# mpeg5/xevd

Hardware: AMD Instinct MI355X
Metric: frames/sec (bit-exact YUV) + achieved HBM GB/s (higher is better)
Workload: dtype s16; 1 GPU; cfg4_main_8k_10b_ra; width=7680, height=4320, bit_depth=10, batches_resident=4, residual_pass_ahead=True, parallelism=1 stream on 1 GPU

## Files before the change

xevd_amd/csrc/k_inter.hip:

```cpp
#include "xgpu_internal.h"

#include <hip/hip_ext.h>
#include <type_traits>
#include "mc_filters.h"

#define LDS_AS __attribute__((address_space(3)))

#define UW_STRIDE 48
#define UI_STRIDE 40
#define UC_STRIDE 24
#define UCW_STRIDE 32
static_assert(UI_STRIDE <= UW_STRIDE && UC_STRIDE <= UCW_STRIDE, "an intermediate row is not longer than the window row it replaces");
#define UT_L_SAMPLES (40 * UW_STRIDE)
#define UT_C_SAMPLES (3 * 64 * 8)
#define UNI_SAMPLES   (UT_L_SAMPLES + UT_C_SAMPLES)
static_assert(2 * 19 * UCW_STRIDE <= UT_C_SAMPLES, "both chroma windows fit");

__device__ __forceinline__ void wave_lds_sync()
{
    __builtin_amdgcn_fence(__ATOMIC_RELEASE, "wavefront");
    __builtin_amdgcn_wave_barrier();
    __builtin_amdgcn_fence(__ATOMIC_ACQUIRE, "wavefront");
}

// ... 93 lines not shown
                const uint2 a = w[0], b = w[1];
                E[0] = a.x; E[1] = a.y; E[2] = b.x; E[3] = b.y;
            }
            uint2 r;
            if (H) {
                const uint32_t O[3] = { hi_lo(E[1], E[0]), hi_lo(E[2], E[1]), hi_lo(E[3], E[2]) };
                int t[4];
                if (SH && odd) {
                    t[0] = dot2(ch[1], O[1], dot2z(ch[0], O[0]));
                    t[1] = dot2(ch[1], E[2], dot2z(ch[0], E[1]));
                    t[2] = dot2(ch[1], O[2], dot2z(ch[0], O[1]));
                    t[3] = dot2(ch[1], E[3], dot2z(ch[0], E[2]));
                } else {
                    t[0] = dot2(ch[1], E[1], dot2z(ch[0], E[0]));
                    t[1] = dot2(ch[1], O[1], dot2z(ch[0], O[0]));
                    t[2] = dot2(ch[1], E[2], dot2z(ch[0], E[1]));
                    t[3] = dot2(ch[1], O[2], dot2z(ch[0], O[1]));
                }
#pragma unroll
                for (int q = 0; q < 4; q++) { t[q] >>= rg.sh1; if (!V) t[q] = clip3(0, maxv, t[q]); }
                r = make_uint2(pack2(t[0], t[1]), pack2(t[2], t[3]));
            } else {
                if (SH && odd) r = make_uint2(E[1], E[2]);
                else r = make_uint2(hi_lo(E[1], E[0]), hi_lo(E[2], E[1]));
            }
            *(uint2 *)(I + prow * UC_STRIDE + 4 * g) = r;
        }
    }
    wave_lds_sync();
#pragma unroll
    for (int pl = 0; pl < 2; pl++) {
        const int16_t *base = I + (pl * 19 + ((lane >> 3) << 1)) * UC_STRIDE + ((lane & 7) << 1);
        uint32_t *o = pl ? ov : ou;
        if (!V) {
            o[0] = *(const uint32_t *)(base + UC_STRIDE); o[1] = *(const uint32_t *)(base + 2 * UC_STRIDE);
        } else {
            uint32_t q[5];
#pragma unroll
            for (int j = 0; j < 5; j++) q[j] = *(const uint32_t *)(base + j * UC_STRIDE);
            int acc[2][2];
#pragma unroll
            for (int j = 1; j < 5; j++) {
                const uint32_t pr[2] = { __builtin_amdgcn_perm(q[j], q[j - 1], 0x05040100u), __builtin_amdgcn_perm(q[j], q[j - 1], 0x07060302u) };
#pragma unroll
                for (int c = 0; c < 2; c++)
#pragma unroll
                    for (int r = 0; r < 2; r++) {
                        const int d = j - 1 - r;
                        if (d == 0) acc[r][c] = dot2a(cv[0], pr[c], rg.off2);
                        else if (d == 2) acc[r][c] = dot2(cv[1], pr[c], acc[r][c]);
                    }
            }
#pragma unroll
            for (int r = 0; r < 2; r++)
                o[r] = pack2(clip3(0, maxv, acc[r][0] >> rg.sh2), clip3(0, maxv, acc[r][1] >> rg.sh2));
        }
    }
    wave_lds_sync();
}
#define REG_W_STRIDE 80
#define REG_C_STRIDE 48
#define REG_W_SAMPLES (71 * REG_W_STRIDE)
#define REG_C_SAMPLES (35 * REG_C_STRIDE)
#define REG_I_SAMPLES (39 * UI_STRIDE)
#define REG_SAMPLES   (REG_W_SAMPLES + 2 * REG_C_SAMPLES + 4 * REG_I_SAMPLES)
struct RegionMap { int y[3], c[2]; };
__device__ __forceinline__ RegionMap region_map(int t)
{
    RegionMap m;
#pragma unroll
    for (int it = 0; it < 3; it++) {
        const int idx = t + 256 * it, row = idx / 10, k = idx - row * 10;
        m.y[it] = idx < 71 * 10 ? (row << 8) | k : -1;
    }
#pragma unroll
    for (int it = 0; it < 2; it++) {
        const int idx = t + 256 * it, pl = idx >= 210, j = idx - 210 * pl, row = j / 6, k = j - row * 6;
        m.c[it] = idx < 420 ? (row << 8) | (pl << 7) | k : -1;
    }
    return m;
}

template <bool H, bool V>
__device__ __forceinline__ void mc_scu_list(gs16 pl_, int s_l, gs16 pu_, gs16 pv_, int s_c, const uint32_t ch[4], const uint32_t cv[4], Regime rgl, int maxl,
                                            const uint32_t c2h[2], const uint32_t c2v[2], Regime rgc, int maxc, bool cwh, bool cwv, uint32_t o[8], uint32_t ou[2], uint32_t ov[2],
                                            bool fx, bool fy, bool cfx, bool cfy)
{
    constexpr int J0 = V ? 0 : 3, J1 = V ? 11 : 7;
#ifdef XGPU_NO_LANE_PRED
    fx = fy = cfx = cfy = true;
#endif
    v4u32 A[11]; v2u32 B[11];
    auto request = [&](int ja, int jb) {
#pragma unroll
        for (int j = ja; j < jb; j++) {
            const bool row_on = !V || fy || (j >= 3 && j < 7);
            if (H) {
                A[j] = any_value<v4u32>(); B[j] = any_value<v2u32>();
                gload16_if(A[j], pl_ + j * s_l, row_on);
                gload8_if(B[j], pl_ + j * s_l + 8, row_on && fx);
            } else {
                B[j] = any_value<v2u32>();
                gload8_if(B[j], pl_ + j * s_l + 3, row_on);
            }
        }
    };
    auto fence = [&](int ja, int jb) {
#pragma unroll
        for (int j = ja; j < jb; j++) {
            if (H) asm volatile("" : "+v"(A[j]), "+v"(B[j]));
            else   asm volatile("" : "+v"(B[j]));
        }
    };
    int acc[4][4];
    int tp[4] = {0, 0, 0, 0};
    auto row = [&](int j) {
        int t[4];
        if (H) {
            const uint32_t D0 = A[j].x, D1 = A[j].y, D2 = A[j].z, D3 = A[j].w, D4 = B[j].x, D5 = B[j].y;
            const uint32_t Q0 = hi_lo(D1, D0), Q1 = hi_lo(D2, D1), Q2 = hi_lo(D3, D2), Q3 = hi_lo(D4, D3), Q4 = hi_lo(D5, D4);
            t[0] = dot2(ch[3], D3, dot2(ch[2], D2, dot2(ch[1], D1, dot2z(ch[0], D0))));
            t[2] = dot2(ch[3], D4, dot2(ch[2], D3, dot2(ch[1], D2, dot2z(ch[0], D1))));
            t[1] = dot2(ch[3], Q3, dot2(ch[2], Q2, dot2(ch[1], Q1, dot2z(ch[0], Q0))));
            t[3] = dot2(ch[3], Q4, dot2(ch[2], Q3, dot2(ch[1], Q2, dot2z(ch[0], Q1))));
#pragma unroll
            for (int c = 0; c < 4; c++) t[c] = clip3(rgl.lo1, rgl.hi1, t[c] >> rgl.sh1);
        } else {
            t[0] = (int)(int16_t)(B[j].x & 0xFFFF); t[1] = (int)(int16_t)(B[j].x >> 16);
            t[2] = (int)(int16_t)(B[j].y & 0xFFFF); t[3] = (int)(int16_t)(B[j].y >> 16);
        }
        if (!V) {
#pragma unroll
            for (int c = 0; c < 4; c++) acc[j - 3][c] = t[c];
            return;
        }
        if (j > 0) {
#pragma unroll
            for (int c = 0; c < 4; c++) {
                const uint32_t pr = pack2(tp[c], t[c]);
#pragma unroll
                for (int r = 0; r < 4; r++) {
                    const int d = j - 1 - r;
                    if (d == 0) acc[r][c] = dot2a(cv[0], pr, rgl.off2);
                    else if (d > 0 && d <= 6 && (d & 1) == 0) acc[r][c] = dot2(cv[d >> 1], pr, acc[r][c]);
                }
            }
        }
#pragma unroll
        for (int c = 0; c < 4; c++) tp[c] = t[c];
    };
    auto rows = [&](int ja, int jb) {
#pragma unroll
        for (int j = ja; j < jb; j++) row(j);
    };
    auto luma_out = [&]() {
#pragma unroll
        for (int r = 0; r < 4; r++) {
            int v[4];
#pragma unroll
            for (int c = 0; c < 4; c++) v[c] = clip3(0, maxl, V ? acc[r][c] >> rgl.sh2 : acc[r][c]);
            o[r * 2 + 0] = pack2(v[0], v[1]);
            o[r * 2 + 1] = pack2(v[2], v[3]);
        }
    };
    v3u32 CW[2][5];
    auto request_c = [&](int pl) {
#pragma unroll
        for (int j = 0; j < 5; j++) {
            const bool row_on = cfy || j == 1 || j == 2;
            CW[pl][j] = any_value<v3u32>();
            gload12_if(CW[pl][j], (pl ? pv_ : pu_) + j * s_c, row_on);
        }
    };
    auto fence_c = [&](int pl) {
#pragma unroll
        for (int j = 0; j < 5; j++) asm volatile("" : "+v"(CW[pl][j]));
    };
    auto chroma = [&](auto hc, auto vc, int pl, uint32_t oo[2]) {
        constexpr bool CH = decltype(hc)::value, CV = decltype(vc)::value;
        int a2[2][2];
        int tq[2] = {0, 0};
#pragma unroll
        for (int j = CV ? 0 : 1; j < (CV ? 5 : 3); j++) {
            int t[2];
            const uint32_t D0 = CW[pl][j].x, D1 = CW[pl][j].y, D2 = CW[pl][j].z;
            if (CH) {
                const uint32_t Q0 = hi_lo(D1, D0), Q1 = hi_lo(D2, D1);
                t[0] = dot2(c2h[1], D1, dot2z(c2h[0], D0));
                t[1] = dot2(c2h[1], Q1, dot2z(c2h[0], Q0));
#pragma unroll
                for (int c = 0; c < 2; c++) t[c] = clip3(rgc.lo1, rgc.hi1, t[c] >> rgc.sh1);
            } else {
                const uint32_t q = hi_lo(D1, D0);
                t[0] = (int)(int16_t)(q & 0xFFFF); t[1] = (int)(int16_t)(q >> 16);
            }
            if (!CV) { a2[j - 1][0] = t[0]; a2[j - 1][1] = t[1]; continue; }
            if (j > 0) {
#pragma unroll
                for (int c = 0; c < 2; c++) {
                    const uint32_t pr = pack2(tq[c], t[c]);
#pragma unroll
                    for (int r = 0; r < 2; r++) {
                        const int d = j - 1 - r;
                        if (d == 0) a2[r][c] = dot2a(c2v[0], pr, rgc.off2);
                        else if (d == 2) a2[r][c] = dot2(c2v[1], pr, a2[r][c]);
                    }
                }
            }
            tq[0] = t[0]; tq[1] = t[1];
        }
#pragma unroll
        for (int r = 0; r < 2; r++)
            oo[r] = pack2(clip3(0, maxc, CV ? a2[r][0] >> rgc.sh2 : a2[r][0]), clip3(0, maxc, CV ? a2[r][1] >> rgc.sh2 : a2[r][1]));
    };
    using T = std::true_type; using F = std::false_type;
    auto chroma_pl = [&](int pl, uint32_t oo[2]) {
        fence_c(pl);
        if (cwh) { if (cwv) chroma(T{}, T{}, pl, oo); else chroma(T{}, F{}, pl, oo); }
        else     { if (cwv) chroma(F{}, T{}, pl, oo); else chroma(F{}, F{}, pl, oo); }
    };
    request(J0, J1); fence(J0, J1);
    rows(J0, J1);
    luma_out();
    __builtin_amdgcn_sched_barrier(0);
    request_c(0); request_c(1);
    chroma_pl(0, ou); chroma_pl(1, ov);
}

#define OWNER_NONE 0xFFFFFFFFu

#ifdef XGPU_INTER_TRACE
__device__ unsigned long long g_inter_trace[3][16];
struct InterTrace { unsigned long long prev; int role; bool on; };
#define TRACE_MARK(tr, p) do { if ((tr).on) { const unsigned long long now_ = __builtin_amdgcn_s_memtime(); atomicAdd(&g_inter_trace[(tr).role][p], now_ - (tr).prev); (tr).prev = __builtin_amdgcn_s_memtime(); } } while (0)
#define TRACE_ARG , InterTrace &tr
#define TRACE_PASS , tr
#define TRACE_OFF InterTrace tr = { 0, 0, false };
extern "C" int xgpu_test_inter_trace(unsigned long long out[48], int reset)
{
    if (hipMemcpyFromSymbol(out, HIP_SYMBOL(g_inter_trace), sizeof(g_inter_trace)) != hipSuccess) return -1;
    if (reset) { static unsigned long long z[48]; if (hipMemcpyToSymbol(HIP_SYMBOL(g_inter_trace), z, sizeof(z)) != hipSuccess) return -1; }
    return 0;
}
#else
#define TRACE_MARK(tr, p) do { } while (0)
#define TRACE_ARG
#define TRACE_PASS
#define TRACE_OFF
#endif
template <int MODE>
__device__ __forceinline__ bool inter_tile(const InterArgs &a, uint4 r0, uint4 r1, bool lane_ok, int sx, int sy, int lane, int16_t *W, const LaneMap fm,
                                           const uint4 (*s_ref)[2], const uint4 *s_ltap, const uint2 *s_ctap, uint32_t pl[8], uint32_t pu[2], uint32_t pv[2],
                                           const RegionMap *rm, int wave, uint32_t own TRACE_ARG)
{
    constexpr bool UNI = MODE != 0;
    if (UNI) {
        own = (uint32_t)__builtin_amdgcn_readfirstlane((int)own);
        r0.x = __builtin_amdgcn_readfirstlane(r0.x); r0.y = __builtin_amdgcn_readfirstlane(r0.y); r0.z = __builtin_amdgcn_readfirstlane(r0.z); r0.w = __builtin_amdgcn_readfirstlane(r0.w);
        r1.x = __builtin_amdgcn_readfirstlane(r1.x); r1.y = __builtin_amdgcn_readfirstlane(r1.y); r1.z = __builtin_amdgcn_readfirstlane(r1.z); r1.w = __builtin_amdgcn_readfirstlane(r1.w);
    } else if (!lane_ok) return false;
    const int cu_x = r0.x & 0xFFFF, cu_y = r0.x >> 16;
    const int lw = r0.y & 0xFF, lh = (r0.y >> 8) & 0xFF, pred_mode = (r0.y >> 16) & 0xF, cbf = r0.y >> 24;
    const int refi0 = (int)(int8_t)(r0.z & 0xFF), refi1 = (int)(int8_t)((r0.z >> 8) & 0xFF), qp_map = (r0.z >> 16) & 0xFF;
    const uint32_t coef_off = r0.w;
    const int cw = 1 << lw, chh = 1 << lh;
    const int x = sx << 2, y = sy << 2;
    const bool intra = pred_mode == XGPU_MODE_INTRA;
    const int ai = (intra || pred_mode == XGPU_MODE_IBC) ? 0 : (int)((r1.w >> 8) & 0xFF);
    int tu_x = 0, tu_y = 0, tu_w = cw, tu_h = chh;
    if (ai) {
        const int idx = ai & 15, pos = ai >> 4;
        if (idx == 2 || idx == 4) { tu_h = chh >> (idx == 4 ? 2 : 1); tu_y = pos ? chh - tu_h : 0; }
        else                      { tu_w = cw >> (idx == 3 ? 2 : 1);  tu_x = pos ? cw - tu_w : 0; }
    }
    const int lx = x - cu_x - tu_x, ly = y - cu_y - tu_y;
    const bool in_tu = (uint32_t)lx < (uint32_t)tu_w && (uint32_t)ly < (uint32_t)tu_h;

    {
        uint32_t m = ((uint32_t)qp_map << 16) | ((uint32_t)intra << 15) | (1u << 31);
        m |= SCU_RANK(own);
        if (pred_mode == XGPU_MODE_SKIP) m |= 1u << 23;
        const bool ibc = pred_mode == XGPU_MODE_IBC;
        if (ibc) m |= 1u << 26;
        if (((r0.z >> 24) & 1) && in_tu) m |= 1u << 24;
        if (((x - cu_x) & 63) == 0) m |= SCU_EDGE_L;
        if (((y - cu_y) & 63) == 0) m |= SCU_EDGE_T;
        if (x == cu_x && ((r0.y >> 16) & CU_NOCH_L)) m |= SCU_NOCH_L;
        if (y == cu_y && ((r0.y >> 16) & CU_NOCH_T)) m |= SCU_NOCH_T;
        uint4 rec;
        rec.x = m;
        rec.y = (intra || ibc) ? 0x0000FFFFu : ((r0.z & 0xFFFFu) | ((uint32_t)ai << 16));
        rec.z = intra ? 0u : r1.x;
        rec.w = (intra || ibc) ? 0u : r1.y;
        bool other0 = false, other1 = false;
        if (!intra && !ibc) {
            if ((r1.w >> 16) & 0xFF) { other0 = refi0 >= 0; other1 = refi1 >= 0; }
            else if (a.dmvr_to_map && (r1.w >> 24)) {
                const int q0 = refi0 >= 0 ? (int)s_ref[refi0 * 2][1].z : 0, q1 = refi1 >= 0 ? (int)s_ref[refi1 * 2 + 1][1].z : 0;
                other0 = other1 = dmvr_applies(a.cur_poc, q0, q1);
            }
        }
        ScuRec *const mp = &a.maps[sy * a.w_scu + sx];
        if (!other0 && !other1) *(uint4 *)mp = rec;
        else {
            *(uint2 *)mp = make_uint2(rec.x, rec.y);
            if (!other0) ((uint32_t *)mp)[2] = rec.z;
// ... 109 lines not shown
                    const int idx = lane + 64 * it, plane = idx >= 76, j = idx - 76 * plane;
                    if (idx < 152 && wanted(j >> 2, j & 3)) __builtin_amdgcn_global_load_lds((const GAS void *)((plane ? rv_ : ru_) + off + (j >> 2) * a.s_c + 8 * (j & 3)), (LDS_AS void *)(d + it * 1024), 16, 0, 0);
                }
            }
        };
        constexpr int N_LUMA_REQ = REGION ? 3 : 4, N_CHROMA_REQ = REGION ? 2 : 3;
        const int l_first = use[0] ? 0 : 1, n_lists = (int)use[0] + (int)use[1];
        TRACE_MARK(tr, 2);
        load_resid();
        if (n_lists) { request_luma(l_first); __builtin_amdgcn_sched_barrier(0); request_chroma(l_first); }
        TRACE_MARK(tr, 3);
#pragma unroll 1
        for (int i = 0; i < n_lists; i++) {
            const int l = i ? 1 : l_first;
            const bool more = i + 1 < n_lists;
            int px, py;
            list_pos(l, px, py);
            const int mvx = l ? mvs[1][0] : mvs[0][0], mvy = l ? mvs[1][1] : mvs[0][1];
            const int ldx = (mvx & 3) != 0, ldy = (mvy & 3) != 0, cdx = (mvx & 7) != 0, cdy = (mvy & 7) != 0;
            uint32_t o[8], ou[2], ov[2];
            if (REGION) { asm volatile("s_waitcnt vmcnt(0)" ::: "memory"); __syncthreads(); }
            else { asm volatile("s_waitcnt vmcnt(%0)" :: "n"(N_CHROMA_REQ) : "memory"); wave_lds_sync(); }
            TRACE_MARK(tr, i ? 8 : 4);
            {
                const uint4 th = s_ltap[ldx ? ((px & 3) << 2) : 16], tv = s_ltap[ldy ? ((py & 3) << 2) : 16];
                const uint32_t ch[4] = { th.x, th.y, th.z, th.w }, cv[4] = { tv.x, tv.y, tv.z, tv.w };
                const Regime rg = regime(ldx, ldy, a.bd_l);
                const int mis = ((px >> 2) - 3) & 7, odd = mis & 1;
                const int16_t *const Wy = Wy0 + (mis & ~1);
                if (ldx) { if (ldy) luma_tile_filter<true, true, WS_L, true>(Wy, ch, cv, rg, maxl, I, lane, o, odd); else luma_tile_filter<true, false, WS_L, true>(Wy, ch, cv, rg, maxl, I, lane, o, odd); }
                else     { if (ldy) luma_tile_filter<false, true, WS_L, true>(Wy, ch, cv, rg, maxl, I, lane, o, odd); else luma_tile_filter<false, false, WS_L, true>(Wy, ch, cv, rg, maxl, I, lane, o, odd); }
            }
            TRACE_MARK(tr, 5);
            if (more) {
                if (REGION) __syncthreads(); else wave_lds_sync();
                request_luma(1);
            }
            if (!REGION) {
                if (more) asm volatile("s_waitcnt vmcnt(%0)" :: "n"(N_LUMA_REQ) : "memory"); else asm volatile("s_waitcnt vmcnt(0)" ::: "memory");
                wave_lds_sync();
            }
            TRACE_MARK(tr, 6);
            {
                const uint2 th = s_ctap[cdx ? ((px & 7) << 2) : 32], tv = s_ctap[cdy ? ((py & 7) << 2) : 32];
                const uint32_t c2h[2] = { th.x, th.y }, c2v[2] = { tv.x, tv.y };
                const Regime rg = regime(cdx, cdy, a.bd_c);
                const int mis = ((px >> 3) - 1) & 7, odd = mis & 1;
                const int16_t *const Wu = Wu0 + (mis & ~1), *const Wv = Wu + C_SAMPLES;
                if (cdx) { if (cdy) chroma_tile_filter<true, true, WS_C, true>(Wu, Wv, c2h, c2v, rg, maxc, IC, lane, ou, ov, odd); else chroma_tile_filter<true, false, WS_C, true>(Wu, Wv, c2h, c2v, rg, maxc, IC, lane, ou, ov, odd); }
                else     { if (cdy) chroma_tile_filter<false, true, WS_C, true>(Wu, Wv, c2h, c2v, rg, maxc, IC, lane, ou, ov, odd); else chroma_tile_filter<false, false, WS_C, true>(Wu, Wv, c2h, c2v, rg, maxc, IC, lane, ou, ov, odd); }
            }
            TRACE_MARK(tr, 7);
            if (more) {
                if (REGION) __syncthreads(); else wave_lds_sync();
                request_chroma(1);
            }
            if (nl == 0) {
#pragma unroll
                for (int k = 0; k < 8; k++) pl[k] = o[k];
                pu[0] = ou[0]; pu[1] = ou[1]; pv[0] = ov[0]; pv[1] = ov[1];
            } else {
#pragma unroll
                for (int k = 0; k < 8; k++) pl[k] = avg2(pl[k], o[k]);
                pu[0] = avg2(pu[0], ou[0]); pu[1] = avg2(pu[1], ou[1]);
                pv[0] = avg2(pv[0], ov[0]); pv[1] = avg2(pv[1], ov[1]);
            }
            nl++;
        }
        (void)tid;
    } else {
        TRACE_MARK(tr, 2);
#pragma unroll
        for (int l = 0; l < 2; l++) {
            if (!use[l]) continue;
            const uint4 e0 = s_ref[refis[l] * 2 + l][0], e1 = s_ref[refis[l] * 2 + l][1];
            const gs16 ry_ = (gs16)(((uint64_t)e0.y << 32) | e0.x), ru_ = (gs16)(((uint64_t)e0.w << 32) | e0.z), rv_ = (gs16)(((uint64_t)e1.y << 32) | e1.x);
            const int mvx = mvs[l][0], mvy = mvs[l][1];
            const int px = (x << 2) + mvt[l][0], py = (y << 2) + mvt[l][1];
            const int ldx = (mvx & 3) != 0, ldy = (mvy & 3) != 0;
            const int cdx = (mvx & 7) != 0, cdy = (mvy & 7) != 0;
            uint32_t ch[4], cv[4], o[8], ou[2], ov[2];
            {
                const uint4 th = s_ltap[ldx ? ((px & 3) << 2) : 16], tv = s_ltap[ldy ? ((py & 3) << 2) : 16];
                ch[0] = th.x; ch[1] = th.y; ch[2] = th.z; ch[3] = th.w; cv[0] = tv.x; cv[1] = tv.y; cv[2] = tv.z; cv[3] = tv.w;
                const uint2 cth = s_ctap[cdx ? ((px & 7) << 2) : 32], ctv = s_ctap[cdy ? ((py & 7) << 2) : 32];
                const uint32_t c2h[2] = { cth.x, cth.y }, c2v[2] = { ctv.x, ctv.y };
                const gs16 p = ry_ + ((py >> 2) - 3) * a.s_l + (px >> 2) - 3;
                const int off = ((py >> 3) - 1) * a.s_c + (px >> 3) - 1;
                const Regime rgl = regime(ldx, ldy, a.bd_l), rgc = regime(cdx, cdy, a.bd_c);
                const bool wh = __ballot(ldx) != 0, wvv = __ballot(ldy) != 0;
                const bool cwh = __ballot(cdx) != 0, cwv = __ballot(cdy) != 0;
#define MC_S(H, V) mc_scu_list<H, V>(p, a.s_l, ru_ + off, rv_ + off, a.s_c, ch, cv, rgl, maxl, c2h, c2v, rgc, maxc, cwh, cwv, o, ou, ov, ldx != 0, ldy != 0, cdx != 0, cdy != 0)
                if (wh) { if (wvv) MC_S(true, true); else MC_S(true, false); }
                else    { if (wvv) MC_S(false, true); else MC_S(false, false); }
#undef MC_S
            }
            if (nl == 0) {
#pragma unroll
                for (int k = 0; k < 8; k++) pl[k] = o[k];
                pu[0] = ou[0]; pu[1] = ou[1]; pv[0] = ov[0]; pv[1] = ov[1];
            } else {
#pragma unroll
                for (int k = 0; k < 8; k++) pl[k] = avg2(pl[k], o[k]);
                pu[0] = avg2(pu[0], ou[0]); pu[1] = avg2(pu[1], ou[1]);
                pv[0] = avg2(pv[0], ov[0]); pv[1] = avg2(pv[1], ov[1]);
            }
            nl++;
        }
    }
    TRACE_MARK(tr, 9);
    if (MODE == 0) load_resid();
    if (nl == 0) return false;

    if (cbf & 1) {
#pragma unroll
        for (int k = 0; k < 8; k++) pl[k] = recon2(pl[k], rl[k], maxl);
    }
    if (cbf & 2) { pu[0] = recon2(pu[0], ru[0], maxl); pu[1] = recon2(pu[1], ru[1], maxl); }
    if (cbf & 4) { pv[0] = recon2(pv[0], rv[0], maxl); pv[1] = recon2(pv[1], rv[1], maxl); }

    return true;
}

__device__ __forceinline__ int xcd_slice(int block, int grid) { return (block & 7) * (grid >> 3) + (block >> 3); }

__device__ __forceinline__ void store_scu(const InterArgs &a, int sx, int sy, const uint32_t pl[8], const uint32_t pu[2], const uint32_t pv[2])
{
    const int x = sx << 2, y = sy << 2;
    int16_t *dy = a.cur_y + y * a.s_l + x;
#pragma unroll
    for (int k = 0; k < 4; k++) *(uint2 *)(dy + k * a.s_l) = make_uint2(pl[k * 2], pl[k * 2 + 1]);
    const int coff = (y >> 1) * a.s_c + (x >> 1);
    *(uint32_t *)(a.cur_u + coff) = pu[0];
    *(uint32_t *)(a.cur_u + coff + a.s_c) = pu[1];
    *(uint32_t *)(a.cur_v + coff) = pv[0];
    *(uint32_t *)(a.cur_v + coff + a.s_c) = pv[1];
}
#define ARG_REFS(a)  ((const uint4 (*)[2])&(a).refp[0][0])
#define ARG_LTAPS(a) ((const uint4 *)&k_luma_taps[(a).admvp][0][0])
#define ARG_CTAPS(a) ((const uint2 *)&k_chroma_taps[(a).admvp][0][0])
static_assert(sizeof(RefEntry) == 32, "a reference entry is two 16-byte halves");
static_assert(XGPU_INTER_STRIP == 16, "the strip arithmetic below shifts by four");

struct SplitTables { uint4 ref[XGPU_MAX_REFS * 2][2]; uint4 ltap[17]; uint2 ctap[33]; uint2 pad; };

__device__ __forceinline__ void inter_fused_body(const InterArgs &a)
{
    __shared__ __attribute__((aligned(16))) int16_t s_win[REG_SAMPLES];
    static_assert(4 * UNI_SAMPLES <= REG_SAMPLES, "the four waves' tile blocks fit into the region block");
    __shared__ SplitTables s_tab[4];
    const int idx = xcd_slice(blockIdx.x, gridDim.x);
    if (idx >= a.n_work) return;
    const int t = threadIdx.x, lane = t & 63, wave = __builtin_amdgcn_readfirstlane(t >> 6);
#ifdef XGPU_INTER_TRACE
    InterTrace tr = { __builtin_amdgcn_s_memtime(), 0, lane == 0 && (idx % 61) == 7 };
#endif
    int rx, ry;
    if (idx < a.full_entries) {
        const int s = (int)__umulhi((uint32_t)idx, a.magic_strip), r = idx - s * a.strip_entries;
        ry = r >> 4; rx = (s << 4) + (r & 15);
    } else {
        const int r = idx - a.full_entries;
        ry = a.magic_last ? (int)__umulhi((uint32_t)r, a.magic_last) : r; rx = (a.regions_x & ~15) + r - ry * (a.regions_x & 15);
    }
    const int sx = (rx << 4) + ((wave & 1) << 3) + (lane & 7), sy = (ry << 4) + ((wave >> 1) << 3) + (lane >> 3);
    const uint32_t kinds = a.work[idx];
    const uint4 *const item = (const uint4 *)&a.items[idx * 4 + wave];
    const uint4 e = item[0], i0 = item[1], i1 = item[2];
    const uint32_t own = (sx < (a.pic_w >> 2) && sy < (a.pic_h >> 2)) ? a.owner[sy * a.w_scu + sx] : OWNER_NONE;
    const LaneMap fm0 = { 0, 0 };
    uint32_t pl[8], pu[2], pv[2];
    if (kinds == XGPU_WORK_REGION) {
// ... 117 lines not shown
```

xevd_amd/csrc/mc_filters.h:

```cpp
#pragma once
#include "xgpu_internal.h"

typedef short v2s __attribute__((ext_vector_type(2)));
struct __attribute__((packed, aligned(2))) U32x4u { uint32_t a, b, c, d; };
struct __attribute__((packed, aligned(2))) U32x2u { uint32_t a, b; };
struct __attribute__((packed, aligned(2))) U32x1u { uint32_t a; };
#define GAS __attribute__((address_space(1)))
typedef const GAS int16_t *gs16;
typedef uint32_t v4u32 __attribute__((ext_vector_type(4)));
typedef uint32_t v2u32 __attribute__((ext_vector_type(2)));
typedef uint32_t v3u32 __attribute__((ext_vector_type(3)));
typedef v4u32 __attribute__((aligned(2))) v4u32_u;
typedef v2u32 __attribute__((aligned(2))) v2u32_u;
typedef v3u32 __attribute__((aligned(2))) v3u32_u;
typedef uint32_t __attribute__((aligned(2))) u32_u;
__device__ __forceinline__ uint4 gload16(gs16 p) { const v4u32 v = *(const GAS v4u32_u *)p; return make_uint4(v.x, v.y, v.z, v.w); }
__device__ __forceinline__ uint2 gload8(gs16 p) { const v2u32 v = *(const GAS v2u32_u *)p; return make_uint2(v.x, v.y); }
__device__ __forceinline__ uint32_t gload4(gs16 p) { return *(const GAS u32_u *)p; }
template <typename T> __device__ __forceinline__ T any_value() { T v; asm volatile("" : "=v"(v)); return v; }
__device__ __forceinline__ void gload16_if(v4u32 &v, gs16 p, bool on) { if (on) v = *(const GAS v4u32_u *)p; }
__device__ __forceinline__ void gload8_if(v2u32 &v, gs16 p, bool on) { if (on) v = *(const GAS v2u32_u *)p; }
__device__ __forceinline__ void gload12_if(v3u32 &v, gs16 p, bool on) { if (on) v = *(const GAS v3u32_u *)p; }
__device__ __forceinline__ void gload4_if(uint32_t &v, gs16 p, bool on) { if (on) v = *(const GAS u32_u *)p; }

__device__ __forceinline__ int dot2(uint32_t a, uint32_t b, int c)
{
    return __builtin_amdgcn_sdot2(__builtin_bit_cast(v2s, a), __builtin_bit_cast(v2s, b), c, false);
}
__device__ __forceinline__ int dot2z(uint32_t a, uint32_t b)
{
    int r;
    asm("v_dot2_i32_i16 %0, %1, %2, 0" : "=v"(r) : "v"(a), "v"(b));
    return r;
}
__device__ __forceinline__ int dot2a(uint32_t a, uint32_t b, int c)
{
    int r;
    asm("v_dot2_i32_i16 %0, %1, %2, %3" : "=v"(r) : "v"(a), "v"(b), "v"(c));
    return r;
}
__device__ __forceinline__ uint32_t hi_lo(uint32_t hi, uint32_t lo)
{
    return __builtin_amdgcn_alignbit(hi, lo, 16);
}
__device__ __forceinline__ uint32_t pack2(int lo, int hi)
{
    return __builtin_amdgcn_perm((uint32_t)hi, (uint32_t)lo, 0x05040100u);
}
__device__ __forceinline__ int clip3(int lo, int hi, int v)
{
    int r;
    asm("v_med3_i32 %0, %1, %2, %3" : "=v"(r) : "v"(v), "v"(lo), "v"(hi));
    return r;
}

#define PK(a, b) ((uint32_t)(uint16_t)(int16_t)(a) | ((uint32_t)(uint16_t)(int16_t)(b) << 16))
#define L8(a, b, c, d, e, f, g, h) { PK(a, b), PK(c, d), PK(e, f), PK(g, h) }
#define C4(a, b, c, d) { PK(a, b), PK(c, d) }
static __constant__ uint32_t k_luma_taps[2][17][4] = {
    { L8(0,0,0,64,0,0,0,0), L8(0,0,0,0,0,0,0,0), L8(0,0,0,0,0,0,0,0), L8(0,0,0,0,0,0,0,0),
      L8(0,1,-5,52,20,-5,1,0), L8(0,0,0,0,0,0,0,0), L8(0,0,0,0,0,0,0,0), L8(0,0,0,0,0,0,0,0),
      L8(0,2,-10,40,40,-10,2,0), L8(0,0,0,0,0,0,0,0), L8(0,0,0,0,0,0,0,0), L8(0,0,0,0,0,0,0,0),
      L8(0,1,-5,20,52,-5,1,0), L8(0,0,0,0,0,0,0,0), L8(0,0,0,0,0,0,0,0), L8(0,0,0,0,0,0,0,0),
      L8(0,0,0,1,0,0,0,0) },
    { L8(0,0,0,64,0,0,0,0), L8(0,1,-3,63,4,-2,1,0), L8(-1,2,-5,62,8,-3,1,0), L8(-1,3,-8,60,13,-4,1,0),
      L8(-1,4,-10,58,17,-5,1,0), L8(-1,4,-11,52,26,-8,3,-1), L8(-1,3,-9,47,31,-10,4,-1), L8(-1,4,-11,45,34,-10,4,-1),
      L8(-1,4,-11,40,40,-11,4,-1), L8(-1,4,-10,34,45,-11,4,-1), L8(-1,4,-10,31,47,-9,3,-1), L8(-1,3,-8,26,52,-11,4,-1),
      L8(0,1,-5,17,58,-10,4,-1), L8(0,1,-4,13,60,-8,3,-1), L8(0,1,-3,8,62,-5,2,-1), L8(0,1,-2,4,63,-3,1,0),
      L8(0,0,0,1,0,0,0,0) },
};
static __constant__ uint32_t k_chroma_taps[2][33][2] = {
    { C4(0,64,0,0), C4(0,0,0,0), C4(0,0,0,0), C4(0,0,0,0), C4(-2,58,10,-2), C4(0,0,0,0), C4(0,0,0,0), C4(0,0,0,0),
      C4(-4,52,20,-4), C4(0,0,0,0), C4(0,0,0,0), C4(0,0,0,0), C4(-6,46,30,-6), C4(0,0,0,0), C4(0,0,0,0), C4(0,0,0,0),
      C4(-8,40,40,-8), C4(0,0,0,0), C4(0,0,0,0), C4(0,0,0,0), C4(-6,30,46,-6), C4(0,0,0,0), C4(0,0,0,0), C4(0,0,0,0),
      C4(-4,20,52,-4), C4(0,0,0,0), C4(0,0,0,0), C4(0,0,0,0), C4(-2,10,58,-2), C4(0,0,0,0), C4(0,0,0,0), C4(0,0,0,0),
      C4(0,1,0,0) },
    { C4(0,64,0,0), C4(-1,63,2,0), C4(-2,62,4,0), C4(-2,60,7,-1), C4(-2,58,10,-2), C4(-3,57,12,-2), C4(-4,56,14,-2), C4(-4,55,15,-2),
      C4(-4,54,16,-2), C4(-5,53,18,-2), C4(-6,52,20,-2), C4(-6,49,24,-3), C4(-6,46,28,-4), C4(-5,44,29,-4), C4(-4,42,30,-4), C4(-4,39,33,-4),
      C4(-4,36,36,-4), C4(-4,33,39,-4), C4(-4,30,42,-4), C4(-4,29,44,-5), C4(-4,28,46,-6), C4(-3,24,49,-6), C4(-2,20,52,-6), C4(-2,18,53,-5),
      C4(-2,16,54,-4), C4(-2,15,55,-4), C4(-2,14,56,-4), C4(-2,12,57,-3), C4(-2,10,58,-2), C4(-1,7,60,-2), C4(0,4,62,-2), C4(0,2,63,-1),
      C4(0,1,0,0) },
};

__device__ __forceinline__ bool dmvr_applies(int poc_c, int poc0, int poc1)
{
    return (poc_c - poc0) * (poc_c - poc1) < 0 && abs(poc_c - poc0) == abs(poc_c - poc1);
}

struct Regime { int sh1, lo1, hi1, sh2, off2; };
__device__ __forceinline__ Regime regime(int has_dx, int has_dy, int bd)
{
    Regime r;
    const int shift1 = min(4, bd - 8), shift2 = max(8, 20 - bd);
    r.sh1   = has_dx ? (has_dy ? shift1 : 6) : 0;
    r.lo1   = (has_dx && !has_dy) ? 0 : (int)0x80000000;
    r.hi1   = (has_dx && !has_dy) ? (1 << bd) - 1 : 0x7FFFFFFF;
    r.sh2   = has_dy ? (has_dx ? shift2 : 6) : 0;
    r.off2  = (has_dy && has_dx) ? (1 << (shift2 - 1)) : 0;
    return r;
}

template <bool H, bool V>
__device__ __forceinline__ void mc_luma_4x4(gs16 p, int s, const uint32_t ch[4], const uint32_t cv[4],
                                            Regime rg, int maxv, uint32_t o[8])
{
    int acc[4][4];
    int tp[4] = {0, 0, 0, 0};
#pragma unroll
    for (int j = V ? 0 : 3; j < (V ? 11 : 7); j++) {
        int t[4];
        if (H) {
            const uint4 a = gload16(p + j * s);
            const uint2 b = gload8(p + j * s + 8);
            const uint32_t D0 = a.x, D1 = a.y, D2 = a.z, D3 = a.w, D4 = b.x, D5 = b.y;
            const uint32_t Q0 = hi_lo(D1, D0), Q1 = hi_lo(D2, D1), Q2 = hi_lo(D3, D2), Q3 = hi_lo(D4, D3), Q4 = hi_lo(D5, D4);
            t[0] = dot2(ch[3], D3, dot2(ch[2], D2, dot2(ch[1], D1, dot2z(ch[0], D0))));
            t[2] = dot2(ch[3], D4, dot2(ch[2], D3, dot2(ch[1], D2, dot2z(ch[0], D1))));
            t[1] = dot2(ch[3], Q3, dot2(ch[2], Q2, dot2(ch[1], Q1, dot2z(ch[0], Q0))));
            t[3] = dot2(ch[3], Q4, dot2(ch[2], Q3, dot2(ch[1], Q2, dot2z(ch[0], Q1))));
#pragma unroll
            for (int c = 0; c < 4; c++) t[c] = clip3(rg.lo1, rg.hi1, t[c] >> rg.sh1);
        } else {
            const uint2 a = gload8(p + j * s + 3);
            t[0] = (int)(int16_t)(a.x & 0xFFFF); t[1] = (int)(int16_t)(a.x >> 16);
            t[2] = (int)(int16_t)(a.y & 0xFFFF); t[3] = (int)(int16_t)(a.y >> 16);
        }
        if (!V) {
#pragma unroll
            for (int c = 0; c < 4; c++) acc[j - 3][c] = t[c];
            continue;
        }
        if (j > 0) {
#pragma unroll
            for (int c = 0; c < 4; c++) {
                const uint32_t pr = pack2(tp[c], t[c]);
#pragma unroll
                for (int r = 0; r < 4; r++) {
                    const int d = j - 1 - r;
                    if (d == 0) acc[r][c] = dot2a(cv[0], pr, rg.off2);
                    else if (d > 0 && d <= 6 && (d & 1) == 0) acc[r][c] = dot2(cv[d >> 1], pr, acc[r][c]);
                }
            }
        }
#pragma unroll
        for (int c = 0; c < 4; c++) tp[c] = t[c];
    }
#pragma unroll
    for (int r = 0; r < 4; r++) {
        int v[4];
#pragma unroll
        for (int c = 0; c < 4; c++) v[c] = clip3(0, maxv, V ? acc[r][c] >> rg.sh2 : acc[r][c]);
        o[r * 2 + 0] = pack2(v[0], v[1]);
        o[r * 2 + 1] = pack2(v[2], v[3]);
    }
}

template <bool H, bool V>
__device__ __forceinline__ void mc_chroma_2x2(gs16 p, int s, const uint32_t ch[2], const uint32_t cv[2],
                                              Regime rg, int maxv, uint32_t o[2])
{
    int acc[2][2];
    int tp[2] = {0, 0};
#pragma unroll
    for (int j = V ? 0 : 1; j < (V ? 5 : 3); j++) {
        int t[2];
        if (H) {
            const v3u32 a = *(const GAS v3u32_u *)(p + j * s);
            const uint32_t D0 = a.x, D1 = a.y, D2 = a.z;
            const uint32_t Q0 = hi_lo(D1, D0), Q1 = hi_lo(D2, D1);
            t[0] = dot2(ch[1], D1, dot2z(ch[0], D0));
            t[1] = dot2(ch[1], Q1, dot2z(ch[0], Q0));
#pragma unroll
            for (int c = 0; c < 2; c++) t[c] = clip3(rg.lo1, rg.hi1, t[c] >> rg.sh1);
        } else {
            const uint32_t a = gload4(p + j * s + 1);
            t[0] = (int)(int16_t)(a & 0xFFFF); t[1] = (int)(int16_t)(a >> 16);
        }
        if (!V) { acc[j - 1][0] = t[0]; acc[j - 1][1] = t[1]; continue; }
        if (j > 0) {
#pragma unroll
            for (int c = 0; c < 2; c++) {
                const uint32_t pr = pack2(tp[c], t[c]);
#pragma unroll
                for (int r = 0; r < 2; r++) {
                    const int d = j - 1 - r;
                    if (d == 0) acc[r][c] = dot2a(cv[0], pr, rg.off2);
                    else if (d == 2) acc[r][c] = dot2(cv[1], pr, acc[r][c]);
                }
            }
        }
        tp[0] = t[0]; tp[1] = t[1];
    }
#pragma unroll
    for (int r = 0; r < 2; r++)
        o[r] = pack2(clip3(0, maxv, V ? acc[r][0] >> rg.sh2 : acc[r][0]), clip3(0, maxv, V ? acc[r][1] >> rg.sh2 : acc[r][1]));
}

typedef unsigned short v2us __attribute__((ext_vector_type(2)));
__device__ __forceinline__ uint32_t avg2(uint32_t a, uint32_t b)
{
    const v2us r = (__builtin_bit_cast(v2us, a) + __builtin_bit_cast(v2us, b) + (v2us)(1)) >> (v2us)(1);
    return __builtin_bit_cast(uint32_t, r);
}
__device__ __forceinline__ uint32_t recon2(uint32_t pred, uint32_t res, int maxv)
{
    const v2s sum = __builtin_bit_cast(v2s, __builtin_bit_cast(v2us, pred) + __builtin_bit_cast(v2us, res));
    const v2s r = __builtin_elementwise_min(__builtin_elementwise_max(sum, (v2s)(0)), (v2s)((short)maxv));
    return __builtin_bit_cast(uint32_t, r);
}
```

Before: 3439 frames/s.

## Fold MC interpolation shifts into pre-scaled taps and byte-permute extraction

Pre-shifts the luma and chroma filter taps left so that each intermediate result lands in a fixed 16-bit field of the 32-bit accumulator. The per-sample arithmetic shifts, clip3 operations and pack2 calls are then replaced by v_perm byte selects plus a packed 16-bit clamp. Compile-time static_asserts check that the scaled taps and sums stay inside s16/s32 at every supported bit depth, which keeps output bit-exact. This cuts VALU instructions in the mc_scu_list hot path at the cost of more complex coefficient setup per block.

```diff
diff --git a/xevd_amd/csrc/k_inter.hip b/xevd_amd/csrc/k_inter.hip
--- a/xevd_amd/csrc/k_inter.hip
+++ b/xevd_amd/csrc/k_inter.hip
@@ -199,8 +199,8 @@
 }
 
 template <bool H, bool V>
-__device__ __forceinline__ void mc_scu_list(gs16 pl_, int s_l, gs16 pu_, gs16 pv_, int s_c, const uint32_t ch[4], const uint32_t cv[4], Regime rgl, int maxl,
-                                            const uint32_t c2h[2], const uint32_t c2v[2], Regime rgc, int maxc, bool cwh, bool cwv, uint32_t o[8], uint32_t ou[2], uint32_t ov[2],
+__device__ __forceinline__ void mc_scu_list(gs16 pl_, int s_l, gs16 pu_, gs16 pv_, int s_c, const uint32_t ch[4], const uint32_t cv[4], Stage2 s2l, int maxl,
+                                            const uint32_t c2h[2], const uint32_t c2v[2], Stage2 s2c, int maxc, bool cwh, bool cwv, uint32_t o[8], uint32_t ou[2], uint32_t ov[2],
                                             bool fx, bool fy, bool cfx, bool cfy)
 {
     constexpr int J0 = V ? 0 : 3, J1 = V ? 11 : 7;
@@ -232,7 +232,7 @@
     int acc[4][4];
     int tp[4] = {0, 0, 0, 0};
     auto row = [&](int j) {
-        int t[4];
+        int t[4] = {0, 0, 0, 0};
         if (H) {
             const uint32_t D0 = A[j].x, D1 = A[j].y, D2 = A[j].z, D3 = A[j].w, D4 = B[j].x, D5 = B[j].y;
             const uint32_t Q0 = hi_lo(D1, D0), Q1 = hi_lo(D2, D1), Q2 = hi_lo(D3, D2), Q3 = hi_lo(D4, D3), Q4 = hi_lo(D5, D4);
@@ -240,11 +240,6 @@
             t[2] = dot2(ch[3], D4, dot2(ch[2], D3, dot2(ch[1], D2, dot2z(ch[0], D1))));
             t[1] = dot2(ch[3], Q3, dot2(ch[2], Q2, dot2(ch[1], Q1, dot2z(ch[0], Q0))));
             t[3] = dot2(ch[3], Q4, dot2(ch[2], Q3, dot2(ch[1], Q2, dot2z(ch[0], Q1))));
-#pragma unroll
-            for (int c = 0; c < 4; c++) t[c] = clip3(rgl.lo1, rgl.hi1, t[c] >> rgl.sh1);
-        } else {
-            t[0] = (int)(int16_t)(B[j].x & 0xFFFF); t[1] = (int)(int16_t)(B[j].x >> 16);
-            t[2] = (int)(int16_t)(B[j].y & 0xFFFF); t[3] = (int)(int16_t)(B[j].y >> 16);
         }
         if (!V) {
 #pragma unroll
@@ -252,14 +247,21 @@
             return;
         }
         if (j > 0) {
+            uint32_t pr[4];
+            if (H) {
+#pragma unroll
+                for (int c = 0; c < 4; c++) pr[c] = pick_b12(tp[c], t[c]);
+            } else {
+                pr[0] = __builtin_amdgcn_perm(B[j].x, B[j - 1].x, 0x05040100u); pr[1] = __builtin_amdgcn_perm(B[j].x, B[j - 1].x, 0x07060302u);
+                pr[2] = __builtin_amdgcn_perm(B[j].y, B[j - 1].y, 0x05040100u); pr[3] = __builtin_amdgcn_perm(B[j].y, B[j - 1].y, 0x07060302u);
+            }
 #pragma unroll
             for (int c = 0; c < 4; c++) {
-                const uint32_t pr = pack2(tp[c], t[c]);
 #pragma unroll
                 for (int r = 0; r < 4; r++) {
                     const int d = j - 1 - r;
-                    if (d == 0) acc[r][c] = dot2a(cv[0], pr, rgl.off2);
-                    else if (d > 0 && d <= 6 && (d & 1) == 0) acc[r][c] = dot2(cv[d >> 1], pr, acc[r][c]);
+                    if (d == 0) acc[r][c] = H ? dot2a(cv[0], pr[c], s2l.off) : dot2z(cv[0], pr[c]);
+                    else if (d > 0 && d <= 6 && (d & 1) == 0) acc[r][c] = dot2(cv[d >> 1], pr[c], acc[r][c]);
                 }
             }
         }
@@ -273,11 +275,10 @@
     auto luma_out = [&]() {
 #pragma unroll
         for (int r = 0; r < 4; r++) {
-            int v[4];
-#pragma unroll
-            for (int c = 0; c < 4; c++) v[c] = clip3(0, maxl, V ? acc[r][c] >> rgl.sh2 : acc[r][c]);
-            o[r * 2 + 0] = pack2(v[0], v[1]);
-            o[r * 2 + 1] = pack2(v[2], v[3]);
+            if (!H && !V) { o[r * 2 + 0] = clamp2(B[r + 3].x, maxl); o[r * 2 + 1] = clamp2(B[r + 3].y, maxl); continue; }
+            const uint32_t sel = (H && V) ? s2l.sel : MC_SEL_B12;
+            o[r * 2 + 0] = clamp2(__builtin_amdgcn_perm((uint32_t)acc[r][1], (uint32_t)acc[r][0], sel), maxl);
+            o[r * 2 + 1] = clamp2(__builtin_amdgcn_perm((uint32_t)acc[r][3], (uint32_t)acc[r][2], sel), maxl);
         }
     };
     v3u32 CW[2][5];
@@ -297,38 +298,40 @@
         constexpr bool CH = decltype(hc)::value, CV = decltype(vc)::value;
         int a2[2][2];
         int tq[2] = {0, 0};
+        uint32_t qp = 0;
 #pragma unroll
         for (int j = CV ? 0 : 1; j < (CV ? 5 : 3); j++) {
-            int t[2];
+            int t[2] = {0, 0};
+            uint32_t q = 0;
             const uint32_t D0 = CW[pl][j].x, D1 = CW[pl][j].y, D2 = CW[pl][j].z;
             if (CH) {
                 const uint32_t Q0 = hi_lo(D1, D0), Q1 = hi_lo(D2, D1);
                 t[0] = dot2(c2h[1], D1, dot2z(c2h[0], D0));
                 t[1] = dot2(c2h[1], Q1, dot2z(c2h[0], Q0));
-#pragma unroll
-                for (int c = 0; c < 2; c++) t[c] = clip3(rgc.lo1, rgc.hi1, t[c] >> rgc.sh1);
-            } else {
-                const uint32_t q = hi_lo(D1, D0);
-                t[0] = (int)(int16_t)(q & 0xFFFF); t[1] = (int)(int16_t)(q >> 16);
-            }
-            if (!CV) { a2[j - 1][0] = t[0]; a2[j - 1][1] = t[1]; continue; }
+            } else q = hi_lo(D1, D0);
+            if (!CV) {
+                if (CH) { a2[j - 1][0] = t[0]; a2[j - 1][1] = t[1]; } else oo[j - 1] = clamp2(q, maxc);
+                continue;
+            }
             if (j > 0) {
+                const uint32_t pr[2] = { CH ? pick_b12(tq[0], t[0]) : __builtin_amdgcn_perm(q, qp, 0x05040100u), CH ? pick_b12(tq[1], t[1]) : __builtin_amdgcn_perm(q, qp, 0x07060302u) };
 #pragma unroll
                 for (int c = 0; c < 2; c++) {
-                    const uint32_t pr = pack2(tq[c], t[c]);
 #pragma unroll
                     for (int r = 0; r < 2; r++) {
                         const int d = j - 1 - r;
-                        if (d == 0) a2[r][c] = dot2a(c2v[0], pr, rgc.off2);
-                        else if (d == 2) a2[r][c] = dot2(c2v[1], pr, a2[r][c]);
+                        if (d == 0) a2[r][c] = CH ? dot2a(c2v[0], pr[c], s2c.off) : dot2z(c2v[0], pr[c]);
+                        else if (d == 2) a2[r][c] = dot2(c2v[1], pr[c], a2[r][c]);
                     }
                 }
             }
-            tq[0] = t[0]; tq[1] = t[1];
-        }
-#pragma unroll
-        for (int r = 0; r < 2; r++)
-            oo[r] = pack2(clip3(0, maxc, CV ? a2[r][0] >> rgc.sh2 : a2[r][0]), clip3(0, maxc, CV ? a2[r][1] >> rgc.sh2 : a2[r][1]));
+            tq[0] = t[0]; tq[1] = t[1]; qp = q;
+        }
+        if (CH || CV) {
+            const uint32_t sel = (CH && CV) ? s2c.sel : MC_SEL_B12;
+#pragma unroll
+            for (int r = 0; r < 2; r++) oo[r] = clamp2(__builtin_amdgcn_perm((uint32_t)a2[r][1], (uint32_t)a2[r][0], sel), maxc);
+        }
     };
     using T = std::true_type; using F = std::false_type;
     auto chroma_pl = [&](int pl, uint32_t oo[2]) {
@@ -339,6 +342,8 @@
     request(J0, J1); fence(J0, J1);
     rows(J0, J1);
     luma_out();
+#pragma unroll
+    for (int k = 0; k < 8; k++) asm volatile("" : "+v"(o[k]));
     __builtin_amdgcn_sched_barrier(0);
     request_c(0); request_c(1);
     chroma_pl(0, ou); chroma_pl(1, ov);
@@ -614,12 +619,15 @@
             uint32_t ch[4], cv[4], o[8], ou[2], ov[2];
             {
                 const uint4 th = s_ltap[ldx ? ((px & 3) << 2) : 16], tv = s_ltap[ldy ? ((py & 3) << 2) : 16];
-                ch[0] = th.x; ch[1] = th.y; ch[2] = th.z; ch[3] = th.w; cv[0] = tv.x; cv[1] = tv.y; cv[2] = tv.z; cv[3] = tv.w;
+                const int eh = tap_scale_h(ldx, ldy, a.bd_l), ev = tap_scale_v(ldx, ldy, a.bd_l);
+                ch[0] = scale_taps(th.x, eh); ch[1] = scale_taps(th.y, eh); ch[2] = scale_taps(th.z, eh); ch[3] = scale_taps(th.w, eh);
+                cv[0] = scale_taps(tv.x, ev); cv[1] = scale_taps(tv.y, ev); cv[2] = scale_taps(tv.z, ev); cv[3] = scale_taps(tv.w, ev);
                 const uint2 cth = s_ctap[cdx ? ((px & 7) << 2) : 32], ctv = s_ctap[cdy ? ((py & 7) << 2) : 32];
-                const uint32_t c2h[2] = { cth.x, cth.y }, c2v[2] = { ctv.x, ctv.y };
+                const int ceh = tap_scale_h(cdx, cdy, a.bd_c), cev = tap_scale_v(cdx, cdy, a.bd_c);
+                const uint32_t c2h[2] = { scale_taps(cth.x, ceh), scale_taps(cth.y, ceh) }, c2v[2] = { scale_taps(ctv.x, cev), scale_taps(ctv.y, cev) };
                 const gs16 p = ry_ + ((py >> 2) - 3) * a.s_l + (px >> 2) - 3;
                 const int off = ((py >> 3) - 1) * a.s_c + (px >> 3) - 1;
-                const Regime rgl = regime(ldx, ldy, a.bd_l), rgc = regime(cdx, cdy, a.bd_c);
+                const Stage2 rgl = stage2(ldx, ldy), rgc = stage2(cdx, cdy);
                 const bool wh = __ballot(ldx) != 0, wvv = __ballot(ldy) != 0;
                 const bool cwh = __ballot(cdx) != 0, cwv = __ballot(cdy) != 0;
 #define MC_S(H, V) mc_scu_list<H, V>(p, a.s_l, ru_ + off, rv_ + off, a.s_c, ch, cv, rgl, maxl, c2h, c2v, rgc, maxc, cwh, cwv, o, ou, ov, ldx != 0, ldy != 0, cdx != 0, cdy != 0)
diff --git a/xevd_amd/csrc/mc_filters.h b/xevd_amd/csrc/mc_filters.h
--- a/xevd_amd/csrc/mc_filters.h
+++ b/xevd_amd/csrc/mc_filters.h
@@ -2,6 +2,7 @@
 #include "xgpu_internal.h"
 
 typedef short v2s __attribute__((ext_vector_type(2)));
+typedef unsigned short v2us __attribute__((ext_vector_type(2)));
 struct __attribute__((packed, aligned(2))) U32x4u { uint32_t a, b, c, d; };
 struct __attribute__((packed, aligned(2))) U32x2u { uint32_t a, b; };
 struct __attribute__((packed, aligned(2))) U32x1u { uint32_t a; };
@@ -55,32 +56,36 @@
 }
 
 #define PK(a, b) ((uint32_t)(uint16_t)(int16_t)(a) | ((uint32_t)(uint16_t)(int16_t)(b) << 16))
+#define LUMA_TAP_ROWS(L8) { \
+    { L8(0,0,0,64,0,0,0,0), L8(0,0,0,0,0,0,0,0), L8(0,0,0,0,0,0,0,0), L8(0,0,0,0,0,0,0,0), \
+      L8(0,1,-5,52,20,-5,1,0), L8(0,0,0,0,0,0,0,0), L8(0,0,0,0,0,0,0,0), L8(0,0,0,0,0,0,0,0), \
+      L8(0,2,-10,40,40,-10,2,0), L8(0,0,0,0,0,0,0,0), L8(0,0,0,0,0,0,0,0), L8(0,0,0,0,0,0,0,0), \
+      L8(0,1,-5,20,52,-5,1,0), L8(0,0,0,0,0,0,0,0), L8(0,0,0,0,0,0,0,0), L8(0,0,0,0,0,0,0,0), \
+      L8(0,0,0,1,0,0,0,0) }, \
+    { L8(0,0,0,64,0,0,0,0), L8(0,1,-3,63,4,-2,1,0), L8(-1,2,-5,62,8,-3,1,0), L8(-1,3,-8,60,13,-4,1,0), \
+      L8(-1,4,-10,58,17,-5,1,0), L8(-1,4,-11,52,26,-8,3,-1), L8(-1,3,-9,47,31,-10,4,-1), L8(-1,4,-11,45,34,-10,4,-1), \
+      L8(-1,4,-11,40,40,-11,4,-1), L8(-1,4,-10,34,45,-11,4,-1), L8(-1,4,-10,31,47,-9,3,-1), L8(-1,3,-8,26,52,-11,4,-1), \
+      L8(0,1,-5,17,58,-10,4,-1), L8(0,1,-4,13,60,-8,3,-1), L8(0,1,-3,8,62,-5,2,-1), L8(0,1,-2,4,63,-3,1,0), \
+      L8(0,0,0,1,0,0,0,0) }, \
+}
+#define CHROMA_TAP_ROWS(C4) { \
+    { C4(0,64,0,0), C4(0,0,0,0), C4(0,0,0,0), C4(0,0,0,0), C4(-2,58,10,-2), C4(0,0,0,0), C4(0,0,0,0), C4(0,0,0,0), \
+      C4(-4,52,20,-4), C4(0,0,0,0), C4(0,0,0,0), C4(0,0,0,0), C4(-6,46,30,-6), C4(0,0,0,0), C4(0,0,0,0), C4(0,0,0,0), \
+      C4(-8,40,40,-8), C4(0,0,0,0), C4(0,0,0,0), C4(0,0,0,0), C4(-6,30,46,-6), C4(0,0,0,0), C4(0,0,0,0), C4(0,0,0,0), \
+      C4(-4,20,52,-4), C4(0,0,0,0), C4(0,0,0,0), C4(0,0,0,0), C4(-2,10,58,-2), C4(0,0,0,0), C4(0,0,0,0), C4(0,0,0,0), \
+      C4(0,1,0,0) }, \
+    { C4(0,64,0,0), C4(-1,63,2,0), C4(-2,62,4,0), C4(-2,60,7,-1), C4(-2,58,10,-2), C4(-3,57,12,-2), C4(-4,56,14,-2), C4(-4,55,15,-2), \
+      C4(-4,54,16,-2), C4(-5,53,18,-2), C4(-6,52,20,-2), C4(-6,49,24,-3), C4(-6,46,28,-4), C4(-5,44,29,-4), C4(-4,42,30,-4), C4(-4,39,33,-4), \
+      C4(-4,36,36,-4), C4(-4,33,39,-4), C4(-4,30,42,-4), C4(-4,29,44,-5), C4(-4,28,46,-6), C4(-3,24,49,-6), C4(-2,20,52,-6), C4(-2,18,53,-5), \
+      C4(-2,16,54,-4), C4(-2,15,55,-4), C4(-2,14,56,-4), C4(-2,12,57,-3), C4(-2,10,58,-2), C4(-1,7,60,-2), C4(0,4,62,-2), C4(0,2,63,-1), \
+      C4(0,1,0,0) }, \
+}
 #define L8(a, b, c, d, e, f, g, h) { PK(a, b), PK(c, d), PK(e, f), PK(g, h) }
 #define C4(a, b, c, d) { PK(a, b), PK(c, d) }
-static __constant__ uint32_t k_luma_taps[2][17][4] = {
-    { L8(0,0,0,64,0,0,0,0), L8(0,0,0,0,0,0,0,0), L8(0,0,0,0,0,0,0,0), L8(0,0,0,0,0,0,0,0),
-      L8(0,1,-5,52,20,-5,1,0), L8(0,0,0,0,0,0,0,0), L8(0,0,0,0,0,0,0,0), L8(0,0,0,0,0,0,0,0),
-      L8(0,2,-10,40,40,-10,2,0), L8(0,0,0,0,0,0,0,0), L8(0,0,0,0,0,0,0,0), L8(0,0,0,0,0,0,0,0),
-      L8(0,1,-5,20,52,-5,1,0), L8(0,0,0,0,0,0,0,0), L8(0,0,0,0,0,0,0,0), L8(0,0,0,0,0,0,0,0),
-      L8(0,0,0,1,0,0,0,0) },
-    { L8(0,0,0,64,0,0,0,0), L8(0,1,-3,63,4,-2,1,0), L8(-1,2,-5,62,8,-3,1,0), L8(-1,3,-8,60,13,-4,1,0),
-      L8(-1,4,-10,58,17,-5,1,0), L8(-1,4,-11,52,26,-8,3,-1), L8(-1,3,-9,47,31,-10,4,-1), L8(-1,4,-11,45,34,-10,4,-1),
-      L8(-1,4,-11,40,40,-11,4,-1), L8(-1,4,-10,34,45,-11,4,-1), L8(-1,4,-10,31,47,-9,3,-1), L8(-1,3,-8,26,52,-11,4,-1),
-      L8(0,1,-5,17,58,-10,4,-1), L8(0,1,-4,13,60,-8,3,-1), L8(0,1,-3,8,62,-5,2,-1), L8(0,1,-2,4,63,-3,1,0),
-      L8(0,0,0,1,0,0,0,0) },
-};
-static __constant__ uint32_t k_chroma_taps[2][33][2] = {
-    { C4(0,64,0,0), C4(0,0,0,0), C4(0,0,0,0), C4(0,0,0,0), C4(-2,58,10,-2), C4(0,0,0,0), C4(0,0,0,0), C4(0,0,0,0),
-      C4(-4,52,20,-4), C4(0,0,0,0), C4(0,0,0,0), C4(0,0,0,0), C4(-6,46,30,-6), C4(0,0,0,0), C4(0,0,0,0), C4(0,0,0,0),
-      C4(-8,40,40,-8), C4(0,0,0,0), C4(0,0,0,0), C4(0,0,0,0), C4(-6,30,46,-6), C4(0,0,0,0), C4(0,0,0,0), C4(0,0,0,0),
-      C4(-4,20,52,-4), C4(0,0,0,0), C4(0,0,0,0), C4(0,0,0,0), C4(-2,10,58,-2), C4(0,0,0,0), C4(0,0,0,0), C4(0,0,0,0),
-      C4(0,1,0,0) },
-    { C4(0,64,0,0), C4(-1,63,2,0), C4(-2,62,4,0), C4(-2,60,7,-1), C4(-2,58,10,-2), C4(-3,57,12,-2), C4(-4,56,14,-2), C4(-4,55,15,-2),
-      C4(-4,54,16,-2), C4(-5,53,18,-2), C4(-6,52,20,-2), C4(-6,49,24,-3), C4(-6,46,28,-4), C4(-5,44,29,-4), C4(-4,42,30,-4), C4(-4,39,33,-4),
-      C4(-4,36,36,-4), C4(-4,33,39,-4), C4(-4,30,42,-4), C4(-4,29,44,-5), C4(-4,28,46,-6), C4(-3,24,49,-6), C4(-2,20,52,-6), C4(-2,18,53,-5),
-      C4(-2,16,54,-4), C4(-2,15,55,-4), C4(-2,14,56,-4), C4(-2,12,57,-3), C4(-2,10,58,-2), C4(-1,7,60,-2), C4(0,4,62,-2), C4(0,2,63,-1),
-      C4(0,1,0,0) },
-};
+static __constant__ uint32_t k_luma_taps[2][17][4] = LUMA_TAP_ROWS(L8);
+static __constant__ uint32_t k_chroma_taps[2][33][2] = CHROMA_TAP_ROWS(C4);
+#undef L8
+#undef C4
 
 __device__ __forceinline__ bool dmvr_applies(int poc_c, int poc0, int poc1)
 {
@@ -99,6 +104,76 @@
     r.off2  = (has_dy && has_dx) ? (1 << (shift2 - 1)) : 0;
     return r;
 }
+
+constexpr int mc_sh1(int bd) { return bd - 8 < 4 ? bd - 8 : 4; }
+constexpr int mc_sh2(int bd) { return 20 - bd > 8 ? 20 - bd : 8; }
+constexpr int mc_e1(int bd) { return 8 - mc_sh1(bd); }
+constexpr int mc_e2(int bd) { return 16 - mc_sh2(bd); }
+#define MC_E_ONE 2
+#define MC_E_ID  8
+#define MC_SEL_B12 0x06050201u
+#define MC_SEL_B23 0x07060302u
+#define L8(a, b, c, d, e, f, g, h) { a, b, c, d, e, f, g, h }
+#define C4(a, b, c, d) { a, b, c, d }
+static constexpr int k_luma_rows[2][17][8] = LUMA_TAP_ROWS(L8);
+static constexpr int k_chroma_rows[2][33][4] = CHROMA_TAP_ROWS(C4);
+#undef L8
+#undef C4
+constexpr long long mc_floor_shift(long long v, int s) { return v >= 0 ? v >> s : -((-v + (1ll << s) - 1) >> s); }
+template <int R, int N>
+constexpr bool mc_scaled_taps_ok(const int (&rows)[2][R][N], int bd)
+{
+    const long long S16_LO = -32768, S16_HI = 32767, S32_LO = -(1ll << 31), S32_HI = (1ll << 31) - 1, maxv = (1ll << bd) - 1;
+    const int sh1 = mc_sh1(bd), e1 = mc_e1(bd), e2 = mc_e2(bd);
+    for (int t = 0; t < 2; t++) {
+        long long t_lo = 0, t_hi = 0;
+        for (int r = 0; r < R; r++) {
+            long long pos = 0, neg = 0;
+            for (int k = 0; k < N; k++) {
+                const long long c = rows[t][r][k];
+                if (c * (1 << MC_E_ID) < S16_LO || c * (1 << MC_E_ID) > S16_HI) return false;
+                if (c > 0) pos += c; else neg += c;
+            }
+            const long long hi = pos * maxv, lo = neg * maxv;
+            if (hi * (1 << MC_E_ONE) > S32_HI || lo * (1 << MC_E_ONE) < S32_LO) return false;
+            if (mc_floor_shift(hi, 6) > S16_HI || mc_floor_shift(lo, 6) < S16_LO) return false;
+            if (hi * (1ll << e1) > S32_HI || lo * (1ll << e1) < S32_LO) return false;
+            const long long th = mc_floor_shift(hi, sh1), tl = mc_floor_shift(lo, sh1);
+            if (th > S16_HI || tl < S16_LO) return false;
+            if (th > t_hi) t_hi = th;
+            if (tl < t_lo) t_lo = tl;
+        }
+        for (int r = 0; r < R; r++) {
+            long long pos = 0, neg = 0;
+            for (int k = 0; k < N; k++) { const long long c = rows[t][r][k]; if (c > 0) pos += c; else neg += c; }
+            const long long hi = (pos * t_hi + neg * t_lo) * (1ll << e2) + (1ll << 15), lo = (pos * t_lo + neg * t_hi) * (1ll << e2) + (1ll << 15);
+            if (hi > S32_HI || lo < S32_LO) return false;
+            if (mc_floor_shift(hi, 16) > S16_HI || mc_floor_shift(lo, 16) < S16_LO) return false;
+        }
+    }
+    return true;
+}
+static_assert(mc_scaled_taps_ok(k_luma_rows, 8) && mc_scaled_taps_ok(k_luma_rows, 9) && mc_scaled_taps_ok(k_luma_rows, 10) && mc_scaled_taps_ok(k_luma_rows, 11) &&
+              mc_scaled_taps_ok(k_luma_rows, 12), "luma: scaled taps are s16, scaled sums stay inside s32, unclipped results are s16 - at every supported bit depth");
+static_assert(mc_scaled_taps_ok(k_chroma_rows, 8) && mc_scaled_taps_ok(k_chroma_rows, 9) && mc_scaled_taps_ok(k_chroma_rows, 10) && mc_scaled_taps_ok(k_chroma_rows, 11) &&
+              mc_scaled_taps_ok(k_chroma_rows, 12), "chroma: the same");
+static_assert(!mc_scaled_taps_ok(k_luma_rows, 16), "the proof can fail: 16-bit samples leave s16 behind one direction");
+
+__device__ __forceinline__ uint32_t scale_taps(uint32_t taps, int e)
+{
+    return __builtin_bit_cast(uint32_t, __builtin_bit_cast(v2us, taps) << (v2us)((unsigned short)e));
+}
+__device__ __forceinline__ uint32_t pick_b12(int lo, int hi) { return __builtin_amdgcn_perm((uint32_t)hi, (uint32_t)lo, MC_SEL_B12); }
+__device__ __forceinline__ uint32_t pick_b23(int lo, int hi) { return __builtin_amdgcn_perm((uint32_t)hi, (uint32_t)lo, MC_SEL_B23); }
+__device__ __forceinline__ uint32_t clamp2(uint32_t v, int maxv)
+{
+    const v2s r = __builtin_elementwise_min(__builtin_elementwise_max(__builtin_bit_cast(v2s, v), (v2s)(0)), (v2s)((short)maxv));
+    return __builtin_bit_cast(uint32_t, r);
+}
+struct Stage2 { uint32_t sel; int off; };
+__device__ __forceinline__ Stage2 stage2(int has_dx, int has_dy) { Stage2 s; s.sel = (has_dx && has_dy) ? MC_SEL_B23 : MC_SEL_B12; s.off = (has_dx && has_dy) ? 0x8000 : 0; return s; }
+__device__ __forceinline__ int tap_scale_h(int has_dx, int has_dy, int bd) { return has_dx ? (has_dy ? mc_e1(bd) : MC_E_ONE) : MC_E_ID; }
+__device__ __forceinline__ int tap_scale_v(int has_dx, int has_dy, int bd) { return has_dy ? (has_dx ? mc_e2(bd) : MC_E_ONE) : MC_E_ID; }
 
 template <bool H, bool V>
 __device__ __forceinline__ void mc_luma_4x4(gs16 p, int s, const uint32_t ch[4], const uint32_t cv[4],
@@ -196,7 +271,6 @@
         o[r] = pack2(clip3(0, maxv, V ? acc[r][0] >> rg.sh2 : acc[r][0]), clip3(0, maxv, V ? acc[r][1] >> rg.sh2 : acc[r][1]));
 }
 
-typedef unsigned short v2us __attribute__((ext_vector_type(2)));
 __device__ __forceinline__ uint32_t avg2(uint32_t a, uint32_t b)
 {
     const v2us r = (__builtin_bit_cast(v2us, a) + __builtin_bit_cast(v2us, b) + (v2us)(1)) >> (v2us)(1);
```

Measured after the change: 3478 frames/s, median of 6. Within noise of the previous version (+1.1%).
